# paritybit-ai/XFL

Measured on AMD Instinct MI355X. Metric: 2048-bit Paillier encrypts/s (device-resident), higher is better.
Workload: dtype u32; 1 GPU; DJN private-key (CRT) encrypt, obfuscated, precision 7, 1000000 float64 plaintexts/GPU resident in HBM; key_bits=2048, elements_per_gpu=1000000, fixed_base_window_bits=23, fixed_base_window_split=False, parallelism=shard1, table_bytes=193273528320

## Files before the change

__graft_entry__.py:

```python
import os
import sys

ROOT = os.path.dirname(os.path.abspath(__file__))
if ROOT not in sys.path:
    sys.path.insert(0, ROOT)


def build() -> None:
    from xfl_amd import build as b
    b.build()
    from oracle import build as ob
    ob.build()
    import runpy
    for script in ("build.py", "build_redc_block.py"):
        try:
            runpy.run_path(os.path.join(ROOT, "tests", "native", script), run_name="tests_native_build")["build"]()
        except Exception as exc:
            print(f"warning: device self-test harnesses not built ({script}): {exc}", file=sys.stderr)
    import xfl_amd
    from xfl_amd import _native
    _native.lib()


def smoke() -> None:
    import numpy as np

    from oracle import paillier_oracle as O
    from xfl_amd import _native as nat
    from xfl_amd.paillier.utils import getprimeover
    import random
    import math

    rng = random.Random(7)
    while True:
        p, q = getprimeover(1024, rng=rng), getprimeover(1024, rng=rng)
        if p != q and math.gcd(p - 1, q - 1) == 2:
            break
    n = p * q
    x = rng.getrandbits(n.bit_length()) | (1 << (n.bit_length() - 1))
    h = pow(-(x * x), n, n * n)
    dk = nat.DeviceKey(2048, n, p, q, h, device=0)
    ok = O.derive_private(p, q, h)
    vals = np.random.default_rng(0).standard_normal(64) * 10
    ms = [O.encode_element(ok, float(v), 7)[0] for v in vals]
    rs = [rng.randrange(1, ok["djn_exp_bound"]) for _ in vals]
    ct = nat.words_to_ints(dk.encrypt_words(nat.ints_to_words(ms, dk.nw), nat.ints_to_words(rs, dk.rand_words)))
    want = [O.encrypt_m(ok, m, r) for m, r in zip(ms, rs)]
# ... 11 lines not shown
```

xfl_amd/csrc/keyconst.hpp:

```cpp
#pragma once
#include <algorithm>
#include <cstdint>
#include <stdexcept>
#include <utility>
#include <vector>

#include "hostbn.hpp"
#include "keydev.hpp"
#include "rns_layout.hpp"

namespace xhe {

struct ModSpec {
  int S, W;
  int S4() const { return (S + 3) & ~3; }
  BigU R() const { return pow2((size_t)W * S); }
};

struct KeySpec {
  int K;
  bool priv, djn;
  ModSpec mp2, mp2L, mp2X;
  ModSpec mp;
  ModSpec mn2, mn2X;
// ... 194 lines not shown
  }
  if (sq) {
    if (ns >= P_SCHED_MAX) throw std::runtime_error("rns schedule overflow");
    v[P_SCHED + ns++] = sq << 8;
  }
  v[P_NS] = (uint32_t)ns;
  return v;
}
}

using RowF = const uint32_t* KeyDev::*;
using PairF = const uint2* KeyDev::*;
using ModF = ModDev KeyDev::*;
using IntF = int KeyDev::*;

struct Dst {
  RowF w = nullptr;
  PairF d = nullptr;
  ModF m = nullptr;
  const uint32_t* ModDev::*mw = nullptr;
  size_t* off = nullptr;
  Dst(RowF f) : w(f) {}
  Dst(PairF f) : d(f) {}
  Dst(ModF mod, const uint32_t* ModDev::*f) : m(mod), mw(f) {}
  Dst(size_t* o) : off(o) {}
};

struct KeyImage {
  std::vector<uint32_t> words;
  KeyDev kd{};
  int rand_bits = 0, rand_words = 0;
  size_t hM_n2 = 0, hM_p2[2] = {0, 0};
  std::vector<uint32_t> hinvM_p[2];

  void put(const std::vector<uint32_t>& v, Dst dst, size_t min_words = 0) {
    const size_t off = words.size();
    const size_t len = (std::max(v.size(), min_words) + 3) & ~(size_t)3;
    words.resize(off + len, 0u);
    std::copy(v.begin(), v.end(), words.begin() + off);
    if (dst.off) *dst.off = off;
    else binds.push_back({dst, off});
  }
  void put_limbs(const BigU& x, const ModSpec& s, Dst dst) { put(x.to_limbs(s.W, s.S), dst, s.S4()); }
  void put_words(const BigU& x, int nw, Dst dst) {
    std::vector<uint32_t> v(nw);
    x.to_words(v.data(), nw);
    put(v, dst);
  }
  void put_mod(const BigU& M, const ModSpec& s, ModF m, int npow = 0) {
    const BigU R1 = mod(s.R(), M), R2 = mulmod(R1, R1, M), R3 = mulmod(R2, R1, M);
    put_limbs(M, s, {m, &ModDev::N});
    put_limbs(R1, s, {m, &ModDev::R1});
    put_limbs(R2, s, {m, &ModDev::R2});
    put_limbs(R3, s, {m, &ModDev::R3});
    (kd.*m).n0inv = mont_ninv(M.word(0), s.W);
    if (npow <= 0) return;
    std::vector<uint32_t> rows((size_t)npow * s.S4(), 0u);
    BigU x = mod(BigU(1), M);
    for (int j = 0; j < npow; ++j) {
      const std::vector<uint32_t> l = x.to_limbs(s.W, s.S);
      std::copy(l.begin(), l.end(), rows.begin() + (size_t)j * s.S4());
      x = mulmod(x, R1, M);
    }
    put(rows, {m, &ModDev::Rpow});
  }

// ... 180 lines not shown
      const BigU &X = pr[i].X, RX = mod(s.pmd.R(), X), R2 = mulmod(RX, RX, X);
      im.put_limbs(mulmod(mod(pr[i].Y, X), mulmod(R2, R2, X), X), s.pmd, pq::mu[i]);
    }
}

inline void pdigit_constants(KeyImage& im, const KeySpec& s, const Prime& pr, int i) {
  const BigU &X = pr.X, &X2 = pr.X2;
  const DigitMod d(X, s.pd);
  digit_modulus(im, d, X2, pq::dm[i], pq::x_kn2[i], pq::x_rmn[i]);
  im.put(mask_plus_e(X, d.RM, d.s), pq::x_topc[i]);
  im.put_limbs(mulmod(mod(pr.Y, X), mulmod(mulmod(d.RM, d.RM, X), d.RM, X), X), d.s, pq::x_fold[i]);
  const BigU Rx2 = mod(d.R, X2), R2 = mulmod(Rx2, Rx2, X2), R4 = mulmod(R2, R2, X2);
  im.put(digit_pairs(d, mulmod(R4, modinv(mod(s.mp2.R(), X2), X2), X2)), pq::x_dwt[i]);
  im.put(digit_pairs(d, R4), pq::x_dw[i]);
  im.put_limbs(mulmod(pr.h, d.RM, X), d.s, pq::x_hpR[i]);
}

inline void exponent_constants(KeyImage& im, const KeySpec& s, const BigU& n, const Prime (&pr)[2]) {
  im.put_limbs(shl(pr[0].X, 1), s.mp, &KeyDev::p2x_lim);
  im.put_limbs(pr[0].X, s.mp, &KeyDev::p_lim);
  for (int i = 0; i < 2; ++i) {
    const BigU e = mod(n, mul(pr[i].X, sub(pr[i].X, BigU(1))));
    im.kd.*pq::e_bits[i] = (int)e.bits();
    im.put_words(e, s.nw(), pq::e_words[i]);
  }
}

inline std::vector<uint32_t> inverse_base_limbs(const ModSpec& s, const BigU& h, const BigU& P) {
  std::vector<uint32_t> v = mulmod(modinv(mod(h, P), P), mod(s.R(), P), P).to_limbs(s.W, s.S);
  v.resize((size_t)s.S4(), 0u);
  return v;
}

inline KeyImage derive_key_constants(const KeySpec& s, const BigU& n, const BigU* p, const BigU* q, const BigU* h) {
  KeyImage im;
  KeyDev& kd = im.kd;
  kd.K = s.K;
  kd.nw = s.nw();
  kd.n2w = s.n2w();
  kd.priv = s.priv;
  kd.djn = s.djn;
  kd.n_bits = (int)n.bits();
  im.rand_bits = s.djn ? (int)(n.bits() / 2) : (int)n.bits();
  im.rand_words = (im.rand_bits + 31) / 32;
  if (s.djn) {
    kd.win = s.win;
    win_layout(im.rand_bits, s.win, s.priv && s.split, &kd.nwin, &kd.nhi);
  }
  const BigU n2 = mul(n, n);
  n2_constants(im, s, n, n2, s.djn && !s.priv ? h : nullptr);
  if (s.K == 2048) {
    kd.ndig = 1;
    ndigit_constants(im, s, n, n2);
  }
  if (!s.priv) return im;
  Prime pr[2] = {{*p, *q, mul(*p, *p), {}, {}}, {*q, *p, mul(*q, *q), {}, {}}};
  for (Prime& x : pr) x.n = mod(n, x.X2);
  prime2_constants(im, s, pr, h, kd.nwin);
  decrypt_constants(im, s, n, pr);
  if (s.K != 2048) {
    kd.pmdx_dec = 1;
    for (int i = 0; i < 2; ++i) pdigit_constants(im, s, pr[i], i);
  }
  exponent_constants(im, s, n, pr);
  if (s.K == 2048 && s.djn)
    for (int i = 0; i < 2; ++i) im.hinvM_p[i] = inverse_base_limbs(s.pmd, *h, pr[i].X);
  return im;
}

}
```

xfl_amd/csrc/pdigit_dev.hpp:

```cpp
#pragma once
#include "bn_dev.hpp"

namespace xhe {

struct PmdLdsQ {
  const uint32_t* q;
  XHE_DEV uint4 load4(int i) const { return *reinterpret_cast<const uint4*>(q + (i >> 2) * 256); }
};

template <int K_>
struct PMD {
  static constexpr int K = K_, W = 28, BL = 6;
  static constexpr int NQ = (2 * K + 3) / 4;
  static constexpr uint32_t MASK = (1u << W) - 1u;
  static_assert((K - 1) % BL == 0, "positions 1..K-1 in blocks of 6");
  static_assert((double)(3 * K + 2) * (double)(1ull << 57) < 18446744073709551616.0, "accumulator bound");

  uint32_t p[K];
  uint32_t n0inv;

  XHE_DEV void init(const uint32_t* __restrict__ P, uint32_t ninv) {
#pragma unroll
    for (int j = 0; j < K; ++j) p[j] = __builtin_amdgcn_readfirstlane(P[j]);
    n0inv = ninv;
// ... 532 lines not shown
  for (int j = 0; j < K; ++j) br = ((int64_t)r[j] - (int64_t)M.p[j] + br) >> 28;
  const bool ge = br == 0;
  br = 0;
#pragma unroll
  for (int j = 0; j < K; ++j) {
    const int64_t v = (int64_t)r[j] - (int64_t)(ge ? M.p[j] : 0u) + br;
    r[j] = (uint32_t)v & ((1u << 28) - 1u);
    br = v >> 28;
  }
  return ge;
}

template <int K>
XHE_DEV void pmd_mod_small(const PMD<K>& M, uint32_t (&m)[K]) {
  constexpr uint32_t MASK = PMD<K>::MASK;
  const uint32_t mt = (m[K - 1] << 4) | (m[K - 2] >> 24);
  const uint32_t pt = (M.p[K - 1] << 4) | (M.p[K - 2] >> 24);
  const uint32_t q = mt / (pt + 1u);
  uint64_t cy = 0;
  int64_t br = 0;
#pragma unroll
  for (int j = 0; j < K; ++j) {
    const uint64_t qp = (uint64_t)q * M.p[j] + cy;
    cy = qp >> 28;
    const int64_t v = (int64_t)m[j] - (int64_t)(qp & MASK) + br;
    m[j] = (uint32_t)v & MASK;
    br = v >> 28;
  }
#pragma unroll
  for (int t = 0; t < 3; ++t) pmd_csub<K>(M, m);
}

template <int K>
XHE_DEV void pmd_from_mont2(const PMD<K>& M, const uint32_t (&X)[2 * K], const uint32_t* RmodP, uint32_t (&e)[K],
                            uint32_t (&f)[K]) {
  uint32_t m[K];
  {
    uint64_t T[2 * K];
#pragma unroll
    for (int j = 0; j < 2 * K; ++j) T[j] = X[j];
    pmd_redc_wide<K>(M, T, e, m);
  }
  __builtin_amdgcn_sched_barrier(0);
  const bool ge = pmd_csub<K>(M, e);
  __builtin_amdgcn_sched_barrier(0);
  pmd_mod_small<K>(M, m);
  __builtin_amdgcn_sched_barrier(0);
  int64_t br = 0;
#pragma unroll
  for (int j = 0; j < K; ++j) {
    const int64_t v = (int64_t)(ge ? RmodP[j] : 0u) - (int64_t)m[j] + br;
    f[j] = (uint32_t)v & ((1u << 28) - 1u);
    br = v >> 28;
  }
  if (br) {
    int64_t cy = 0;
#pragma unroll
    for (int j = 0; j < K; ++j) {
      const int64_t v = (int64_t)f[j] + (int64_t)M.p[j] + cy;
      f[j] = (uint32_t)v & ((1u << 28) - 1u);
      cy = v >> 28;
    }
  }
}

template <int K, int RW>
// ... 647 lines not shown
```

xfl_amd/csrc/xhe.hip:

```cpp
#include <hip/hip_runtime.h>
#include <stdint.h>
#include <stdlib.h>
#include <string.h>

#include <chrono>
#include <cmath>
#include <cstdio>
#include <memory>
#include <mutex>
#include <atomic>
#include <stdexcept>
#include <unordered_map>
#include <utility>
#include <string>
#include <type_traits>
#include <vector>

#include "../../include/xhe.h"
#include "abi_common.hpp"
#include "hostbn.hpp"
#include "keyconst.hpp"
#include "paths.hpp"
#include "xhe_kernels.hpp"
#include "fermat_dev.hpp"
// ... 132 lines not shown
}

}

struct xhe_key {
  int device = 0;
  int K = 0, nw = 0, n2w = 0;
  bool priv = false, djn = false;
  int rand_bits = 0, rand_words = 0;
  uint32_t* d_blob = nullptr;
  uint32_t* d_tab = nullptr;
  KeyDev kd{};
  std::vector<uint32_t> n_host;
  std::vector<uint32_t> n2_host;
  int n_bits = 0;
  int dneg = 0;
};

namespace {

struct DevGuard {
  int prev = -1;
  explicit DevGuard(int dev) {
    HIPCHK(hipGetDevice(&prev));
    if (prev != dev) HIPCHK(hipSetDevice(dev));
  }
  ~DevGuard() {
    if (prev >= 0) (void)hipSetDevice(prev);
  }
};

template <class MP2, int RW>
void build_tables_m(xhe_key* k, const ModDev& md, const uint32_t* d_hM, uint32_t* d_tab, uint32_t* d_chain,
                    uint32_t* d_ws, hipStream_t s);

int64_t chain_rows_h(int win) { return ((int64_t)1 << (win / 2)) + ((int64_t)1 << (win - win / 2)); }

template <class MP2, int RW>
void build_tables_sync(xhe_key* k, const ModDev* md, const uint32_t* const* d_hM, uint32_t* const* d_tab, int count) {
  hipStream_t st[2] = {nullptr, nullptr};
  uint32_t* ws[2] = {nullptr, nullptr};
  uint32_t* chain[2] = {nullptr, nullptr};
  const int win = k->kd.win, nwin = k->kd.nwin, nhi = k->kd.nhi;
  const size_t chain_words =
      (size_t)std::max<int64_t>(nhi ? (nhi + 1) * chain_rows_h(win + 1) : 0, (nwin - nhi) * chain_rows_h(win)) *
      MP2::S4;
  for (int i = 0; i < count; ++i) {
    HIPCHK(hipStreamCreateWithFlags(&st[i], hipStreamNonBlocking));
    HIPCHK(hipMalloc(&ws[i], MP2::S4 * sizeof(uint32_t) * 4));
    HIPCHK(hipMalloc(&chain[i], chain_words * sizeof(uint32_t)));
    build_tables_m<MP2, RW>(k, md[i], d_hM[i], d_tab[i], chain[i], ws[i], st[i]);
  }
  for (int i = 0; i < count; ++i) {
    HIPCHK(hipStreamSynchronize(st[i]));
    HIPCHK(hipFree(ws[i]));
    HIPCHK(hipFree(chain[i]));
    HIPCHK(hipStreamDestroy(st[i]));
  }
}

template <class MP2>
void build_chains_seg(const ModDev& md, const uint32_t* d_base, int win, int nwin, int nbases, uint32_t* d_chain,
                      uint32_t* d_ws, hipStream_t s) {
  const int half = win / 2;
  launch(k_tab_bases<MP2>, dim3(1), dim3(64), s, md, d_base, win, nbases, d_chain, d_ws);
  auto blocks = [&](int64_t groups) { return dim3((unsigned)std::max<int64_t>(1, (groups * MP2::TPI + 255) / 256)); };
  launch(k_tab_one<MP2>, blocks(nwin), dim3(256), s, md, win, nwin, d_chain);
  const int lim_lo = (1 << half) + 1, lim_hi = 1 << (win - half);
  for (int t = 0; (1 << t) < lim_lo - 1; ++t) {
    launch(k_tab_level<MP2>, blocks((int64_t)nwin << t), dim3(256), s, md, md.N, win, nwin, t, 0, lim_lo, d_chain);
  }
  for (int t = 0; (1 << t) < lim_hi - 1; ++t) {
    launch(k_tab_level<MP2>, blocks((int64_t)nwin << t), dim3(256), s, md, md.N, win, nwin, t, half, lim_hi, d_chain);
  }
}

template <class MP2, int RW>
void build_tables_seg(const ModDev& md, const uint32_t* d_base, int win, int nwin, int nbases, uint32_t* d_tab,
                      int64_t rs, uint32_t* d_chain, uint32_t* d_ws, hipStream_t s) {
  build_chains_seg<MP2>(md, d_base, win, nwin, nbases, d_chain, d_ws, s);
  auto blocks = [&](int64_t groups) { return dim3((unsigned)std::max<int64_t>(1, (groups * MP2::TPI + 255) / 256)); };
  int64_t rows = (int64_t)nwin << win;
  launch((k_tab_combine<MP2, RW>), blocks(rows), dim3(256), s, md, md.N, win, nwin, d_chain, d_tab, rs);
}

template <class MP2, int RW>
void build_tables_m(xhe_key* k, const ModDev& md, const uint32_t* d_hM, uint32_t* d_tab, uint32_t* d_chain,
                    uint32_t* d_ws, hipStream_t s) {
  const int win = k->kd.win, nwin = k->kd.nwin, nhi = k->kd.nhi;
  const int64_t rs = RW == k->K / 32 ? k->kd.tab_rs : RW;
  if (nhi == 0) {
    build_tables_seg<MP2, RW>(md, d_hM, win, nwin, nwin, d_tab, rs, d_chain, d_ws, s);
    return;
  }
  uint32_t* base2 = d_ws + 2 * MP2::S4;
  build_tables_seg<MP2, RW>(md, d_hM, win + 1, nhi, nhi + 1, d_tab, rs, d_chain, d_ws, s);
  HIPCHK(hipMemcpyAsync(base2, d_chain + ((size_t)nhi * chain_rows_h(win + 1) + 1) * MP2::S4,
                        MP2::S4 * sizeof(uint32_t), hipMemcpyDeviceToDevice, s));
  build_tables_seg<MP2, RW>(md, base2, win, nwin - nhi, nwin - nhi, d_tab + ((size_t)nhi << (win + 1)) * rs, rs,
                            d_chain, d_ws, s);
}

template <class M>
size_t inv_chain_words(const KeyDev& kd) {
  return (size_t)(kd.nhi * chain_rows_h(kd.win + 1) + (kd.nwin - kd.nhi) * chain_rows_h(kd.win)) * M::S4;
}
template <class M>
void build_chains_m(const KeyDev& kd, const ModDev& md, const uint32_t* d_hM, uint32_t* d_chain, uint32_t* d_ws,
                    hipStream_t s) {
  const int win = kd.win, nwin = kd.nwin, nhi = kd.nhi;
  if (nhi == 0) {
    build_chains_seg<M>(md, d_hM, win, nwin, nwin, d_chain, d_ws, s);
    return;
  }
  uint32_t* base2 = d_ws + 2 * M::S4;
  uint32_t* narrow = d_chain + (size_t)nhi * chain_rows_h(win + 1) * M::S4;
  build_chains_seg<M>(md, d_hM, win + 1, nhi, nhi + 1, d_chain, d_ws, s);
  HIPCHK(hipMemcpyAsync(base2, narrow + M::S4, M::S4 * sizeof(uint32_t), hipMemcpyDeviceToDevice, s));
  build_chains_seg<M>(md, base2, win, nwin - nhi, nwin - nhi, narrow, d_ws, s);
}

template <class Sh>
KeySpec key_spec(const xhe_key* k, int win) {
  KeySpec s{};
  s.K = Sh::K;
  s.priv = k->priv;
  s.djn = k->djn;
  s.win = win & 0xff;
  s.split = (win & XHE_WIN_SPLIT) != 0;
  s.mp2 = {Sh::MP2::S, Sh::MP2::W};
  s.mp2L = {Sh::MP2L::S, Sh::MP2L::W};
  s.mp2X = {Sh::MP2X::S, Sh::MP2X::W};
  s.mp = {Sh::MP::S, Sh::MP::W};
// ... 14 lines not shown
  return s;
}

int64_t table_rows(const KeyDev& kd) { return (int64_t)(kd.nwin + kd.nhi) << kd.win; }

template <class F>
void rows_to_digits(int64_t rows, int tpr, unsigned block, int ntab, F&& launch_one) {
  const dim3 grid((unsigned)((rows * tpr + block - 1) / block));
  for (int i = 0; i < ntab; ++i) launch_one(i, grid, dim3(block));
  HIPCHK(hipDeviceSynchronize());
}

void build_private_tables(xhe_key* k, const KeyImage& im) {
  KeyDev& kd = k->kd;
  const int64_t rows = table_rows(kd);
  const size_t tab_words = (size_t)rows * (size_t)(k->K / 32);
  HIPCHK(hipMalloc(&k->d_tab, 2 * tab_words * sizeof(uint32_t)));
  kd.tab_rs = k->K / 32;
  kd.tab_p2 = k->d_tab;
  kd.tab_q2 = k->d_tab + tab_words;
  const ModDev mds[2] = {kd.p2, kd.q2};
  const uint32_t* hms[2] = {k->d_blob + im.hM_p2[0], k->d_blob + im.hM_p2[1]};
  uint32_t* tabs[2] = {k->d_tab, k->d_tab + tab_words};
  with_shape(k->K, [&](auto sh) {
    using Sh = decltype(sh);
    if constexpr (Sh::K == 2048) {
      using MP = typename Sh::MP;
      const ModDev mp[2] = {kd.p, kd.q};
      hipStream_t st[2];
      uint32_t *inv[2], *ws[2];
      for (int i = 0; i < 2; ++i) {
        HIPCHK(hipStreamCreateWithFlags(&st[i], hipStreamNonBlocking));
        HIPCHK(hipMalloc(&inv[i], inv_chain_words<MP>(kd) * sizeof(uint32_t)));
        HIPCHK(hipMalloc(&ws[i], MP::S4 * sizeof(uint32_t) * 4));
        uint32_t* base = ws[i] + 3 * MP::S4;
        HIPCHK(hipMemcpy(base, im.hinvM_p[i].data(), MP::S4 * sizeof(uint32_t), hipMemcpyHostToDevice));
        build_chains_m<MP>(kd, mp[i], base, inv[i], ws[i], st[i]);
      }
      build_tables_sync<typename Sh::MP2, Sh::RW>(k, mds, hms, tabs, 2);
      for (int i = 0; i < 2; ++i) HIPCHK(hipStreamSynchronize(st[i]));
      kd.pmd = 1;
      rows_to_digits(rows, 1, 256, 2, [&](int i, dim3 grid, dim3 block) {
        launch((k_tab_to_pmd<MP, Sh::RW>), grid, block, nullptr, mp[i], mp[i].N, inv[i], kd.win, kd.nhi, tabs[i], rows,
               (int64_t)kd.tab_rs);
      });
      for (int i = 0; i < 2; ++i) {
        HIPCHK(hipFree(inv[i]));
        HIPCHK(hipFree(ws[i]));
        HIPCHK(hipStreamDestroy(st[i]));
      }
    } else {
      build_tables_sync<typename Sh::MP2, Sh::RW>(k, mds, hms, tabs, 2);
      kd.pmdx = 1;
      using D = typename Sh::PDXO;
      rows_to_digits(rows, D::TPI, 128, 2, [&](int i, dim3 grid, dim3 block) {
        launch((k_tab_to_pmdx<D, Sh::RW>), grid, block, nullptr, kd, i, tabs[i], rows, (int64_t)kd.tab_rs);
      });
    }
  });
}

void build_public_tables(xhe_key* k, const KeyImage& im) {
  KeyDev& kd = k->kd;
  const int64_t rows = table_rows(kd);
  HIPCHK(hipMalloc(&k->d_tab, (size_t)rows * (size_t)(k->K / 16) * sizeof(uint32_t)));
  kd.tab_n2 = k->d_tab;
  const uint32_t* hm = k->d_blob + im.hM_n2;
  uint32_t* tab = k->d_tab;
  with_shape(k->K, [&](auto sh) {
    using Sh = decltype(sh);
    build_tables_sync<typename Sh::MN2, Sh::RW2>(k, &kd.n2, &hm, &tab, 1);
    if constexpr (Sh::K == 2048) {
      if (!pins().ndig_pub) return;
      kd.pub_nd = 1;
      rows_to_digits(rows, ND2048::TPI, 128, 1, [&](int, dim3 grid, dim3 block) {
        launch((k_tab_to_pmdx<ND2048, Sh::RW2>), grid, block, nullptr, kd, 2, tab, rows, (int64_t)Sh::RW2);
// ... 195 lines not shown

template <class Sh, class MP2 = typename Sh::MP2>
void crt_enc_launch(const xhe_key* k, int64_t n, uint32_t* ws, uint32_t* ct, hipStream_t s) {
  const int blocks = (int)((n * MP2::TPI + 255) / 256);
  if constexpr (MP2::TPI == 1)
    launch((k_crt_enc_w<MP2, 2 * Sh::K / 32>), dim3(blocks), dim3(256), s, k->kd, k->kd.p2.N, n, ws, ct);
  else
    launch(k_crt_enc<MP2>, dim3(blocks), dim3(256), s, k->kd, k->kd.p2.N, n, ws, ct);
}

template <class Sh>
void encrypt_impl(const xhe_key* k, const uint32_t* m, const uint32_t* r, int64_t count, uint32_t* ct, hipStream_t s) {
  using MP2 = typename Sh::MP2;
  int64_t chunk = std::min<int64_t>(count, kChunk);
  WsScope wsc(s);
  uint32_t* ws = wsc.get<uint32_t>((size_t)2 * 2 * MP2::S4 * chunk * sizeof(uint32_t));
  uint2* xst = nullptr;
  uint32_t *xrows = nullptr, *xwords = nullptr;
  for (int64_t off = 0; off < count; off += chunk) {
    int64_t n = std::min(chunk, count - off);
    switch (paths::enc_djn(Sh::K, MP2::TPI, k->kd.pmd, k->kd.pmdx, n, pins())) {
      case paths::EncDjn::PMD:
        if constexpr (Sh::K == 2048) {
          ProfScope ps("k_djn_pmd", s);
          const int G = paths::pmd_split(n, pins());
          const dim3 grid((unsigned)((n * G + 127) / 128), 2);
          auto run = [&](auto kern) {
            launch(kern, grid, dim3(128), s, k->kd, k->kd.p.N, k->kd.q.N, k->kd.p2.N, k->kd.q2.N,
                   m + (size_t)off * k->nw, r + (size_t)off * k->rand_words, k->rand_words, n, ws);
          };
          if (G == 16) run(k_djn_pmd<MP2, 37, Sh::RW, 16>);
          else if (G == 4) run(k_djn_pmd<MP2, 37, Sh::RW, 4>);
          else run(k_djn_pmd<MP2, 37, Sh::RW, 1>);
          crt_enc_launch<Sh>(k, n, ws, ct + (size_t)off * k->n2w, s);
          continue;
        } else no_path("encrypt (k_djn_pmd)");
      case paths::EncDjn::PMDX:
        if constexpr (Sh::K != 2048) {
          using D = typename Sh::PDX;
          if (!xst) {
            xst = wsc.get<uint2>((size_t)2 * D::K * chunk * sizeof(uint2));
            xrows = wsc.get<uint32_t>((size_t)2 * 2 * Sh::PDXO::MN::S4 * chunk * sizeof(uint32_t));
            xwords = wsc.get<uint32_t>((size_t)2 * chunk * Sh::RW * sizeof(uint32_t));
          }
          const dim3 g4((unsigned)((n * D::TPI + 127) / 128), 2);
          {
            ProfScope ps("k_djn_pmdx", s);
            launch((k_djn_pmdx<D, Sh::RW>), g4, dim3(128), s, k->kd, r + (size_t)off * k->rand_words, k->rand_words, n,
                   xst);
          }
          using DO = typename Sh::PDXO;
          launch((k_pmdx_enc_out<DO, Sh::RW>), dim3((unsigned)((n * DO::TPI + 127) / 128), 2), dim3(128), s, k->kd,
                 m + (size_t)off * k->nw, n, xst, xrows, xwords);
          launch(k_words_to_rows<MP2>, dim3((unsigned)((n * MP2::TPI + 255) / 256), 2), dim3(256), s, xwords, Sh::RW,
                 n, ws);
          crt_enc_launch<Sh>(k, n, ws, ct + (size_t)off * k->n2w, s);
          continue;
        } else no_path("encrypt (k_djn_pmdx)");
      case paths::EncDjn::POW_X: {
        using MX = typename Sh::MP2X;
        launch((k_djn_pow_x<MX, MP2::S4, Sh::RW>), dim3((unsigned)((n * MX::TPI + 255) / 256), 2), dim3(256), s, k->kd,
               m + (size_t)off * k->nw, r + (size_t)off * k->rand_words, k->rand_words, n, ws);
        break;
      }
      case paths::EncDjn::POW_LDS:
        if constexpr (MP2::TPI == 1) {
          ProfScope ps("k_djn_pow_lds", s);
// ... 1702 lines not shown
```

xfl_amd/csrc/xhe_kernels.hpp:

```cpp
#pragma once
#include "bn_dev.hpp"
#include "keydev.hpp"
#include "pdigit_dev.hpp"

#include <type_traits>

namespace xhe {

enum : int32_t { ST_OK = 0, ST_OVERFLOW = 1, ST_VALUE = 2 };

struct EncVal {
  int32_t st, e;
  int neg, w;
  uint32_t v0, v1, v2;
};

XHE_DEV EncVal encode_value(double v, int mode, int e0, int has_max, int max_exp) {
  EncVal r{ST_OK, 0, 0, 0, 0u, 0u, 0u};
  uint64_t bits = __double_as_longlong(v);
  r.neg = (int)(bits >> 63);
  int bexp = (int)((bits >> 52) & 0x7FF);
  uint64_t frac = bits & ((1ull << 52) - 1);
  int e;
  if (mode == 0) {
// ... 530 lines not shown
    }
#pragma unroll
    for (int j = 0; j < KP; ++j) c[j] = 0u;
  }
  for (int w = g + G; w < key.nwin; w += G) {
    stage(w);
    M.mul_row(a, c, slot, topc);
  }
  if constexpr (G > 1) {
#pragma unroll
    for (int s = 1; s < G; s <<= 1) {
      const bool writer = (g & (2 * s - 1)) == s && g < key.nwin;
      const bool reader = (g & (2 * s - 1)) == 0 && g + s < key.nwin;
      if (reader) D::lam_add_slot(slot, slot + 4 * s);
      wave_sync_mem_();
      if (writer) {
#pragma unroll
        for (int q = 0; q < D::NQ; ++q)
          *reinterpret_cast<uint4*>(slot + q * 256) =
              make_uint4(2 * q < KP ? a[2 * q] : 0u, 2 * q < KP ? c[2 * q] : 0u, 2 * q + 1 < KP ? a[2 * q + 1] : 0u,
                         2 * q + 1 < KP ? c[2 * q + 1] : 0u);
      }
      wave_sync_mem_();
      if (reader) M.mul(a, c, slot + 4 * s, topc);
      wave_sync_mem_();
    }
    if (g != 0) return;
  }
  M.finish(a, c, slot, prime ? Pq : Pp);
  __builtin_amdgcn_sched_barrier(0);
  uint32_t b[MP2::L];
  M.to_mont2(a, c, b);
  __builtin_amdgcn_sched_barrier(0);
  MP2 N;
  N.init(prime ? Nq2 : Np2, prime ? key.q2.n0inv : key.p2.n0inv);
  N.redc_wide(b, AZero{});
  N.reduce_once(b);
  const int64_t eo = ((int64_t)blockIdx.x * blockDim.x + (uint32_t)opaque_i((int)threadIdx.x)) / G;
  N.store_strided(b, ws + (size_t)prime * 2 * MP2::S4 * count + eo, (int)count);
}

template <int KP>
XHE_DEV void pmd_pow_uniform(const PMD<KP>& M, uint32_t (&a)[KP], uint32_t (&c)[KP], const uint32_t* ex, int ebits,
                             uint4* __restrict__ tab_base, int lane, int G, uint32_t* slot, const uint32_t* topc) {
  constexpr int NQ = PMD<KP>::NQ;
#define tab (tab_base + opaque_i(lane))
  auto quad = [&](int q) -> uint4 {
    return make_uint4(2 * q < KP ? a[2 * q] : 0u, 2 * q < KP ? c[2 * q] : 0u, 2 * q + 1 < KP ? a[2 * q + 1] : 0u,
                      2 * q + 1 < KP ? c[2 * q + 1] : 0u);
  };
  auto put_slot = [&]() XHE_INL {
#pragma unroll
    for (int q = 0; q < NQ; ++q) *reinterpret_cast<uint4*>(slot + q * 256) = quad(q);
  };
  auto put_tab = [&](int t) XHE_INL {
#pragma unroll
    for (int q = 0; q < NQ; ++q) tab[((size_t)t * NQ + q) * G] = quad(q);
  };
  auto tab_to_slot = [&](int t) XHE_INL {
    uint4 v[NQ];
#pragma unroll
    for (int q = 0; q < NQ; ++q) v[q] = tab[((size_t)t * NQ + q) * G];
#pragma unroll
    for (int q = 0; q < NQ; ++q) *reinterpret_cast<uint4*>(slot + q * 256) = v[q];
  };
  auto tab_to_regs = [&](int t) XHE_INL {
#pragma unroll
    for (int q = 0; q < NQ; ++q) {
      const uint4 v = tab[((size_t)t * NQ + q) * G];
// ... 578 lines not shown
    wave_sync_mem_();
  };
  auto emit = [&](uint32_t limb) XHE_INL {
    acc |= (uint64_t)limb << nb;
    nb += W;
    if (nb >= 32 && w < NW2) {
      ring[lane * RS + (w & 63)] = (uint32_t)acc;
      acc >>= 32;
      nb -= 32;
      ++w;
      if ((w & 31) == 0) flush((w - 32) & 63);
    }
  };
  for (int i0 = 0; i0 < MP2::S4; i0 += 4) {
    const uint4 a4 = ARow{key.q2_lim}.load4(i0);
#pragma unroll
    for (int r = 0; r < 4; ++r) {
      if (i0 + r < S) {
        const uint32_t ai = comp4(a4, r);
        const uint64_t x0 = mad64(ai, b[0], T[0]);
        mad_shift(T, b, ai);
        T[S - 1] = 0;
        T[0] += x0 >> W;
        emit((uint32_t)x0 & MP2::MASK);
      }
    }
  }
  uint32_t hi[S];
  M.normalize(T, hi);
#pragma unroll
  for (int j = 0; j < S; ++j) emit(hi[j]);
}

template <class MP2>
__global__ void __launch_bounds__(256, 2) k_raw_enc(KeyDev key, const uint32_t* __restrict__ m_words, int64_t count,
                                                    uint32_t* __restrict__ ws, uint32_t* __restrict__ out) {
  const int64_t e = ((int64_t)blockIdx.x * blockDim.x + threadIdx.x) / MP2::TPI;
  if (e >= count) return;
  const int st = (int)count;
  uint32_t* row = ws + e;
  MP2 M;
  M.init(key.p2.N, 0);
  uint32_t b[MP2::L];
  M.load_words(b, m_words + (size_t)e * key.nw, key.nw);
  {
    const int g = MP2::G::g();
#pragma unroll
    for (int j = 0; j < MP2::L; ++j) row[(size_t)(g * MP2::L + j) * st] = (g == 0 && j == 0) ? 1u : 0u;
  }
  wave_sync_mem_();
  M.wide_mul_add_store(b, ARow{key.n_lim}, row, st, out + (size_t)e * key.n2w, key.n2w);
}

template <class MP2>
XHE_DEV void pow_uniform_exp(const MP2& M, uint32_t (&b)[MP2::L], const uint32_t* ex, int ebits,
                             uint32_t* tab, uint32_t* sq, int st, uint32_t* sq_lds = nullptr) {
  const size_t rs = (size_t)MP2::S4 * st;
  auto square = [&]() XHE_INL {
    if constexpr (MP2::kSqr) {
      if (sq_lds) {
        M.sqr(b, SqLds<MP2>(sq_lds));
        return;
      }
    }
    if (sq_lds) {
      const SqLds<MP2> L(sq_lds);
// ... 868 lines not shown
  const int w = (int)(((int64_t)blockIdx.x * blockDim.x + threadIdx.x) / MP2::TPI);
  if (w >= nwin) return;
  MP2 M;
  M.init(md.N, md.n0inv);
  uint32_t b[MP2::L];
  M.load_row(b, md.R1);
  M.reduce_once(b);
  M.store_row(b, chain + (size_t)w * chain_rows(win) * MP2::S4);
}

template <class MP2>
__global__ void __launch_bounds__(256, 2) k_tab_level(ModDev md, const uint32_t* __restrict__ Nm, int win, int nwin,
                                                       int t, int sh, int lim, uint32_t* __restrict__ chain) {
  const int64_t idx = ((int64_t)blockIdx.x * blockDim.x + threadIdx.x) / MP2::TPI;
  const int64_t per = (int64_t)1 << t;
  if (idx >= (int64_t)nwin * per) return;
  const int w = (int)(idx >> t);
  const int64_t d = per + 1 + (idx & (per - 1));
  if (d >= lim) return;
  const int half = win / 2;
  uint32_t* cw = chain + (size_t)w * chain_rows(win) * MP2::S4;
  MP2 M;
  M.init(Nm, md.n0inv);
  uint32_t b[MP2::L];
  M.load_row(b, cw + (size_t)chain_index(d - per, sh, half) * MP2::S4);
  M.mul(b, ARow{cw + (size_t)chain_index(per, sh, half) * MP2::S4});
  M.reduce_once(b);
  M.store_row(b, cw + (size_t)chain_index(d, sh, half) * MP2::S4);
}

template <class MP2, int RW>
__global__ void __launch_bounds__(256, 2) k_tab_combine(ModDev md, const uint32_t* __restrict__ Nm, int win,
                                                         int nwin, const uint32_t* __restrict__ chain,
                                                         uint32_t* __restrict__ tab, int64_t rs) {
  __shared__ __attribute__((aligned(16))) uint32_t sc_all[(256 / MP2::TPI) * MP2::S4];
  const int64_t idx = ((int64_t)blockIdx.x * blockDim.x + threadIdx.x) / MP2::TPI;
  const int64_t rows = (int64_t)nwin << win;
  if (idx >= rows) return;
  const int half = win / 2;
  const int w = (int)(idx >> win);
  const int d = (int)(idx & ((1 << win) - 1));
  const int lo = d & ((1 << half) - 1), hi = d >> half;
  const uint32_t* cw = chain + (size_t)w * chain_rows(win) * MP2::S4;
  MP2 M;
  M.init(Nm, md.n0inv);
  uint32_t b[MP2::L];
  if (hi == 0) {
    M.load_row(b, cw + (size_t)chain_index(lo, 0, half) * MP2::S4);
  } else if (lo == 0) {
    M.load_row(b, cw + (size_t)chain_index(hi, half, half) * MP2::S4);
  } else {
    M.load_row(b, cw + (size_t)chain_index(hi, half, half) * MP2::S4);
    M.mul(b, ARow{cw + (size_t)chain_index(lo, 0, half) * MP2::S4});
    M.reduce_once(b);
  }
  uint32_t* sc = sc_all + (size_t)((threadIdx.x % 256) / MP2::TPI) * MP2::S4;
  M.store_row(b, sc);
  wave_sync_mem_();
  pack_words_<MP2::W, MP2::TPI>(sc, 1, MP2::S, tab + (size_t)idx * rs, RW);
}

template <class MP, int RW>
__global__ void __launch_bounds__(256, 2) k_tab_to_pmd(ModDev mp, const uint32_t* __restrict__ P,
                                                       const uint32_t* __restrict__ inv, int win, int nhi,
                                                       uint32_t* __restrict__ tab, int64_t rows, int64_t rs) {
  static_assert(MP::TPI == 1 && MP::W == 28, "one lane per row on the digit limbs");
  constexpr int KP = MP::S;
  const int64_t r = (int64_t)blockIdx.x * blockDim.x + threadIdx.x;
  if (r >= rows) return;
  uint32_t* row = tab + (size_t)r * rs;
  uint32_t w[RW];
#pragma unroll
  for (int q = 0; q < RW / 4; ++q) {
    const uint4 v = reinterpret_cast<const uint4*>(row)[q];
    w[4 * q] = v.x, w[4 * q + 1] = v.y, w[4 * q + 2] = v.z, w[4 * q + 3] = v.w;
  }
  uint32_t X[2 * KP];
#pragma unroll
  for (int l = 0; l < 2 * KP; ++l) {
    const int bit = 28 * l, k = bit >> 5, sh = bit & 31;
    const uint32_t lo = word_or0(w, k, RW), hi = word_or0(w, k + 1, RW);
    X[l] = __builtin_amdgcn_alignbit(hi, lo, sh) & ((1u << 28) - 1u);
  }
  PMD<KP> M;
  M.init(P, mp.n0inv);
  uint32_t e[KP], f[KP];
  pmd_from_mont2<KP>(M, X, mp.R1, e, f);
  __builtin_amdgcn_sched_barrier(0);
  {
    const int64_t wide = (int64_t)nhi << (win + 1);
    const bool hiw = r < wide;
    const int wb = win + (hiw ? 1 : 0), half = wb / 2;
    const int64_t rr = hiw ? r : r - wide;
    const int64_t d = rr & (((int64_t)1 << wb) - 1);
    const uint32_t* cw = inv + ((size_t)(rr >> wb) * chain_rows(wb) + (hiw ? 0 : (size_t)nhi * chain_rows(win + 1))) * MP::S4;
    const int64_t lo = d & (((int64_t)1 << half) - 1), hi = d >> half;
    MP N;
    N.init(P, mp.n0inv);
    N.mul(f, ARow{cw + (size_t)(hi ? chain_index(hi, half, half) : 0) * MP::S4});
    N.reduce_once(f);
    N.mul(f, ARow{cw + (size_t)chain_index(lo, 0, half) * MP::S4});
    N.reduce_once(f);
  }
  auto word = [&](const uint32_t (&l)[KP], int k) -> uint32_t {
    const int bit = 32 * k, j = bit / 28, sh = bit - 28 * j;
    uint64_t v = (uint64_t)l[j] >> sh;
    if (j + 1 < KP) v |= (uint64_t)l[j + 1] << (28 - sh);
    if (j + 2 < KP) v |= (uint64_t)l[j + 2] << (56 - sh);
    return (uint32_t)v;
  };
#pragma unroll
  for (int q = 0; q < RW / 8; ++q) {
    reinterpret_cast<uint4*>(row)[q] = make_uint4(word(e, 4 * q), word(e, 4 * q + 1), word(e, 4 * q + 2), word(e, 4 * q + 3));
    reinterpret_cast<uint4*>(row)[RW / 8 + q] =
        make_uint4(word(f, 4 * q), word(f, 4 * q + 1), word(f, 4 * q + 2), word(f, 4 * q + 3));
  }
}

XHE_DEV void magwin_push(uint32_t w4[4], uint32_t& low_or, int& hk, uint32_t w, int k) {
  if (!w) return;
  const int g = k - hk;
#pragma unroll
  for (int t = 0; t < 4; ++t)
    if (t < g) low_or |= w4[t];
  uint32_t nw4[4];
#pragma unroll
  for (int t = 0; t < 4; ++t) nw4[t] = t == 3 ? w : (t + g <= 3 ? w4[t + g] : 0u);
#pragma unroll
  for (int t = 0; t < 4; ++t) w4[t] = nw4[t];
  hk = k;
}

XHE_DEV void magwin_round53(const uint32_t w4[4], uint32_t low_or, int hk, int bl, bool rne, uint64_t& mant,
                            int& shift) {
  auto magw = [&](int k) -> uint32_t {
// ... 174 lines not shown
```

Before: 51.08 million encrypts/s.

## Fold CRT recombination constants into tables and use symmetric CRT combine kernel

Precomputes CRT coefficients (inverse of the other prime squared) and folds them into the first window row of the fixed-base tables and their inverse digit tables, so the per-residue results already carry the CRT scaling. The per-element Montgomery exit reduction is replaced by a cheap quotient-estimate reduction, and the final CRT recombination becomes a new kernel computing u*q^2 + v*p^2 with a single conditional subtraction of n^2, using LDS staging for coalesced output. The aim is to remove the multiplications and reductions of the old CRT combine. It adds table-build complexity and relies on carefully argued bounds for the partial reductions.

```diff
diff --git a/__graft_entry__.py b/__graft_entry__.py
--- a/__graft_entry__.py
+++ b/__graft_entry__.py
@@ -12,7 +12,7 @@
     from oracle import build as ob
     ob.build()
     import runpy
-    for script in ("build.py", "build_redc_block.py"):
+    for script in ("build.py", "build_redc_block.py", "build_exit_reduce.py"):
         try:
             runpy.run_path(os.path.join(ROOT, "tests", "native", script), run_name="tests_native_build")["build"]()
         except Exception as exc:
diff --git a/xfl_amd/csrc/keyconst.hpp b/xfl_amd/csrc/keyconst.hpp
--- a/xfl_amd/csrc/keyconst.hpp
+++ b/xfl_amd/csrc/keyconst.hpp
@@ -250,6 +250,7 @@
   int rand_bits = 0, rand_words = 0;
   size_t hM_n2 = 0, hM_p2[2] = {0, 0};
   std::vector<uint32_t> hinvM_p[2];
+  std::vector<uint32_t> crtC_p2[2], crtCinv_p[2];
 
   void put(const std::vector<uint32_t>& v, Dst dst, size_t min_words = 0) {
     const size_t off = words.size();
@@ -496,6 +497,15 @@
   return v;
 }
 
+inline void crt_fold_limbs(const KeySpec& s, const Prime& pr, std::vector<uint32_t>& cM, std::vector<uint32_t>& cinvM) {
+  const BigU Y2 = mod(mul(pr.Y, pr.Y), pr.X2);
+  cM = modinv(Y2, pr.X2).to_limbs(s.mp2.W, s.mp2.S);
+  cM.resize((size_t)s.mp2.S4(), 0u);
+  const BigU &X = pr.X, R2 = mod(s.mp2.R(), X), R = mod(s.pmd.R(), X);
+  cinvM = mulmod(mod(Y2, X), mulmod(R2, R, X), X).to_limbs(s.pmd.W, s.pmd.S);
+  cinvM.resize((size_t)s.pmd.S4(), 0u);
+}
+
 inline KeyImage derive_key_constants(const KeySpec& s, const BigU& n, const BigU* p, const BigU* q, const BigU* h) {
   KeyImage im;
   KeyDev& kd = im.kd;
@@ -528,7 +538,10 @@
   }
   exponent_constants(im, s, n, pr);
   if (s.K == 2048 && s.djn)
-    for (int i = 0; i < 2; ++i) im.hinvM_p[i] = inverse_base_limbs(s.pmd, *h, pr[i].X);
+    for (int i = 0; i < 2; ++i) {
+      im.hinvM_p[i] = inverse_base_limbs(s.pmd, *h, pr[i].X);
+      crt_fold_limbs(s, pr[i], im.crtC_p2[i], im.crtCinv_p[i]);
+    }
   return im;
 }
 
diff --git a/xfl_amd/csrc/pdigit_dev.hpp b/xfl_amd/csrc/pdigit_dev.hpp
--- a/xfl_amd/csrc/pdigit_dev.hpp
+++ b/xfl_amd/csrc/pdigit_dev.hpp
@@ -588,6 +588,26 @@
 }
 
 template <int K>
+XHE_DEV void pmd_exit_reduce(uint32_t (&V)[2 * K], const uint32_t* __restrict__ N2) {
+  static_assert(K == 37, "the tops are taken at bit 2016 = 28 * 72 of a 2048-bit P^2");
+  constexpr int S = 2 * K;
+  constexpr uint32_t MASK = PMD<K>::MASK;
+  const uint64_t vt = ((uint64_t)V[S - 1] << 28) | V[S - 2];
+  const uint32_t pt = (N2[S - 1] << 28) | N2[S - 2];
+  const uint32_t qh = (uint32_t)((double)vt / ((double)pt + 1.0));
+  uint64_t cy = 0;
+  int64_t br = 0;
+#pragma unroll
+  for (int j = 0; j < S; ++j) {
+    const uint64_t qp = mad64s(qh, N2[j], cy);
+    cy = qp >> 28;
+    const int64_t v = (int64_t)V[j] - (int64_t)(qp & MASK) + br;
+    V[j] = j + 1 < S ? ((uint32_t)v & MASK) : (uint32_t)v;
+    br = v >> 28;
+  }
+}
+
+template <int K>
 XHE_DEV void pmd_from_mont2(const PMD<K>& M, const uint32_t (&X)[2 * K], const uint32_t* RmodP, uint32_t (&e)[K],
                             uint32_t (&f)[K]) {
   uint32_t m[K];
diff --git a/xfl_amd/csrc/xhe.hip b/xfl_amd/csrc/xhe.hip
--- a/xfl_amd/csrc/xhe.hip
+++ b/xfl_amd/csrc/xhe.hip
@@ -188,12 +188,13 @@
 
 template <class MP2, int RW>
 void build_tables_m(xhe_key* k, const ModDev& md, const uint32_t* d_hM, uint32_t* d_tab, uint32_t* d_chain,
-                    uint32_t* d_ws, hipStream_t s);
+                    uint32_t* d_ws, hipStream_t s, const uint32_t* d_c0);
 
 int64_t chain_rows_h(int win) { return ((int64_t)1 << (win / 2)) + ((int64_t)1 << (win - win / 2)); }
 
 template <class MP2, int RW>
-void build_tables_sync(xhe_key* k, const ModDev* md, const uint32_t* const* d_hM, uint32_t* const* d_tab, int count) {
+void build_tables_sync(xhe_key* k, const ModDev* md, const uint32_t* const* d_hM, uint32_t* const* d_tab, int count,
+                       const uint32_t* const* d_c0 = nullptr) {
   hipStream_t st[2] = {nullptr, nullptr};
   uint32_t* ws[2] = {nullptr, nullptr};
   uint32_t* chain[2] = {nullptr, nullptr};
@@ -205,7 +206,7 @@
     HIPCHK(hipStreamCreateWithFlags(&st[i], hipStreamNonBlocking));
     HIPCHK(hipMalloc(&ws[i], MP2::S4 * sizeof(uint32_t) * 4));
     HIPCHK(hipMalloc(&chain[i], chain_words * sizeof(uint32_t)));
-    build_tables_m<MP2, RW>(k, md[i], d_hM[i], d_tab[i], chain[i], ws[i], st[i]);
+    build_tables_m<MP2, RW>(k, md[i], d_hM[i], d_tab[i], chain[i], ws[i], st[i], d_c0 ? d_c0[i] : nullptr);
   }
   for (int i = 0; i < count; ++i) {
     HIPCHK(hipStreamSynchronize(st[i]));
@@ -233,28 +234,28 @@
 
 template <class MP2, int RW>
 void build_tables_seg(const ModDev& md, const uint32_t* d_base, int win, int nwin, int nbases, uint32_t* d_tab,
-                      int64_t rs, uint32_t* d_chain, uint32_t* d_ws, hipStream_t s) {
+                      int64_t rs, uint32_t* d_chain, uint32_t* d_ws, hipStream_t s, const uint32_t* d_c0) {
   build_chains_seg<MP2>(md, d_base, win, nwin, nbases, d_chain, d_ws, s);
   auto blocks = [&](int64_t groups) { return dim3((unsigned)std::max<int64_t>(1, (groups * MP2::TPI + 255) / 256)); };
   int64_t rows = (int64_t)nwin << win;
-  launch((k_tab_combine<MP2, RW>), blocks(rows), dim3(256), s, md, md.N, win, nwin, d_chain, d_tab, rs);
+  launch((k_tab_combine<MP2, RW>), blocks(rows), dim3(256), s, md, md.N, win, nwin, d_chain, d_tab, rs, d_c0);
 }
 
 template <class MP2, int RW>
 void build_tables_m(xhe_key* k, const ModDev& md, const uint32_t* d_hM, uint32_t* d_tab, uint32_t* d_chain,
-                    uint32_t* d_ws, hipStream_t s) {
+                    uint32_t* d_ws, hipStream_t s, const uint32_t* d_c0) {
   const int win = k->kd.win, nwin = k->kd.nwin, nhi = k->kd.nhi;
   const int64_t rs = RW == k->K / 32 ? k->kd.tab_rs : RW;
   if (nhi == 0) {
-    build_tables_seg<MP2, RW>(md, d_hM, win, nwin, nwin, d_tab, rs, d_chain, d_ws, s);
+    build_tables_seg<MP2, RW>(md, d_hM, win, nwin, nwin, d_tab, rs, d_chain, d_ws, s, d_c0);
     return;
   }
   uint32_t* base2 = d_ws + 2 * MP2::S4;
-  build_tables_seg<MP2, RW>(md, d_hM, win + 1, nhi, nhi + 1, d_tab, rs, d_chain, d_ws, s);
+  build_tables_seg<MP2, RW>(md, d_hM, win + 1, nhi, nhi + 1, d_tab, rs, d_chain, d_ws, s, d_c0);
   HIPCHK(hipMemcpyAsync(base2, d_chain + ((size_t)nhi * chain_rows_h(win + 1) + 1) * MP2::S4,
                         MP2::S4 * sizeof(uint32_t), hipMemcpyDeviceToDevice, s));
   build_tables_seg<MP2, RW>(md, base2, win, nwin - nhi, nwin - nhi, d_tab + ((size_t)nhi << (win + 1)) * rs, rs,
-                            d_chain, d_ws, s);
+                            d_chain, d_ws, s, nullptr);
 }
 
 template <class M>
@@ -335,16 +336,20 @@
       for (int i = 0; i < 2; ++i) {
         HIPCHK(hipStreamCreateWithFlags(&st[i], hipStreamNonBlocking));
         HIPCHK(hipMalloc(&inv[i], inv_chain_words<MP>(kd) * sizeof(uint32_t)));
-        HIPCHK(hipMalloc(&ws[i], MP::S4 * sizeof(uint32_t) * 4));
+        HIPCHK(hipMalloc(&ws[i], (MP::S4 * 5 + Sh::MP2::S4) * sizeof(uint32_t)));
         uint32_t* base = ws[i] + 3 * MP::S4;
         HIPCHK(hipMemcpy(base, im.hinvM_p[i].data(), MP::S4 * sizeof(uint32_t), hipMemcpyHostToDevice));
+        HIPCHK(hipMemcpy(ws[i] + 4 * MP::S4, im.crtCinv_p[i].data(), MP::S4 * sizeof(uint32_t), hipMemcpyHostToDevice));
+        HIPCHK(hipMemcpy(ws[i] + 5 * MP::S4, im.crtC_p2[i].data(), Sh::MP2::S4 * sizeof(uint32_t), hipMemcpyHostToDevice));
         build_chains_m<MP>(kd, mp[i], base, inv[i], ws[i], st[i]);
       }
-      build_tables_sync<typename Sh::MP2, Sh::RW>(k, mds, hms, tabs, 2);
+      const uint32_t* c0[2] = {ws[0] + 5 * MP::S4, ws[1] + 5 * MP::S4};
+      build_tables_sync<typename Sh::MP2, Sh::RW>(k, mds, hms, tabs, 2, c0);
       for (int i = 0; i < 2; ++i) HIPCHK(hipStreamSynchronize(st[i]));
       kd.pmd = 1;
       rows_to_digits(rows, 1, 256, 2, [&](int i, dim3 grid, dim3 block) {
-        launch((k_tab_to_pmd<MP, Sh::RW>), grid, block, nullptr, mp[i], mp[i].N, inv[i], kd.win, kd.nhi, tabs[i], rows,
+        launch((k_tab_to_pmd<MP, Sh::RW>), grid, block, nullptr, mp[i], mp[i].N, inv[i], ws[i] + 4 * MP::S4, kd.win,
+               kd.nhi, tabs[i], rows,
                (int64_t)kd.tab_rs);
       });
       for (int i = 0; i < 2; ++i) {
@@ -606,7 +611,8 @@
           if (G == 16) run(k_djn_pmd<MP2, 37, Sh::RW, 16>);
           else if (G == 4) run(k_djn_pmd<MP2, 37, Sh::RW, 4>);
           else run(k_djn_pmd<MP2, 37, Sh::RW, 1>);
-          crt_enc_launch<Sh>(k, n, ws, ct + (size_t)off * k->n2w, s);
+          launch((k_crt_sym_w<MP2, 2 * Sh::K / 32>), dim3((unsigned)((n + 255) / 256)), dim3(256), s, k->kd,
+                 k->kd.p2.N, k->kd.q2.N, n, ws, ct + (size_t)off * k->n2w);
           continue;
         } else no_path("encrypt (k_djn_pmd)");
       case paths::EncDjn::PMDX:
diff --git a/xfl_amd/csrc/xhe_kernels.hpp b/xfl_amd/csrc/xhe_kernels.hpp
--- a/xfl_amd/csrc/xhe_kernels.hpp
+++ b/xfl_amd/csrc/xhe_kernels.hpp
@@ -586,9 +586,9 @@
   uint32_t b[MP2::L];
   M.to_mont2(a, c, b);
   __builtin_amdgcn_sched_barrier(0);
+  pmd_exit_reduce<KP>(b, prime ? Nq2 : Np2);
   MP2 N;
   N.init(prime ? Nq2 : Np2, prime ? key.q2.n0inv : key.p2.n0inv);
-  N.redc_wide(b, AZero{});
   N.reduce_once(b);
   const int64_t eo = ((int64_t)blockIdx.x * blockDim.x + (uint32_t)opaque_i((int)threadIdx.x)) / G;
   N.store_strided(b, ws + (size_t)prime * 2 * MP2::S4 * count + eo, (int)count);
@@ -1233,6 +1233,115 @@
   for (int j = 0; j < S; ++j) emit(hi[j]);
 }
 
+template <int N>
+XHE_DEV void mad2s_shift6(uint64_t (&T)[N], uint32_t u, uint32_t v, const uint32_t* __restrict__ A,
+                          const uint32_t* __restrict__ B, int j) {
+  asm("v_mad_u64_u32 %0, vcc, %7, %9, %1\n\t"
+      "v_mad_u64_u32 %1, vcc, %7, %10, %2\n\t"
+      "v_mad_u64_u32 %2, vcc, %7, %11, %3\n\t"
+      "v_mad_u64_u32 %3, vcc, %7, %12, %4\n\t"
+      "v_mad_u64_u32 %4, vcc, %7, %13, %5\n\t"
+      "v_mad_u64_u32 %5, vcc, %7, %14, %6\n\t"
+      "v_mad_u64_u32 %0, vcc, %8, %15, %0\n\t"
+      "v_mad_u64_u32 %1, vcc, %8, %16, %1\n\t"
+      "v_mad_u64_u32 %2, vcc, %8, %17, %2\n\t"
+      "v_mad_u64_u32 %3, vcc, %8, %18, %3\n\t"
+      "v_mad_u64_u32 %4, vcc, %8, %19, %4\n\t"
+      "v_mad_u64_u32 %5, vcc, %8, %20, %5"
+      : "+v"(T[j - 1]), "+v"(T[j]), "+v"(T[j + 1]), "+v"(T[j + 2]), "+v"(T[j + 3]), "+v"(T[j + 4])
+      : "v"(T[j + 5]), "v"(u), "v"(v), "s"(A[j]), "s"(A[j + 1]), "s"(A[j + 2]), "s"(A[j + 3]), "s"(A[j + 4]),
+        "s"(A[j + 5]), "s"(B[j]), "s"(B[j + 1]), "s"(B[j + 2]), "s"(B[j + 3]), "s"(B[j + 4]), "s"(B[j + 5])
+      : "vcc");
+}
+
+template <class MP2, int NW2>
+__global__ void __launch_bounds__(256, 2) k_crt_sym_w(KeyDev key, const uint32_t* __restrict__ Np2,
+                                                      const uint32_t* __restrict__ Nq2, int64_t count,
+                                                      const uint32_t* __restrict__ ws, uint32_t* __restrict__ out) {
+  static_assert(MP2::TPI == 1, "one lane per residue");
+  constexpr int S = MP2::S, W = MP2::W, RS = S + 1;
+  static_assert(NW2 % 32 == 0 && 2 * S * W >= 32 * NW2 + 1, "ciphertext words and the bit above them");
+  static_assert(S >= 64 && (RS & 1) == 1, "the ring (64 words) inside a lane's row; odd stride: no bank conflicts");
+  static_assert((S - 2) % 6 == 0, "positions 1..S-2 in blocks of 6, position S-1 alone");
+  static_assert((double)(2 * S) * (double)((1ull << W) - 1) * (double)((1ull << W) - 1) + (double)(1ull << (64 - W)) <
+                    18446744073709551616.0,
+                "column bound: 2 S products and a carry");
+  __shared__ uint32_t img_all[4][64 * RS];
+  const int64_t e = (int64_t)blockIdx.x * blockDim.x + threadIdx.x;
+  const int lane = (int)(threadIdx.x & 63);
+  uint32_t* ring = img_all[(threadIdx.x >> 6) & 3];
+  uint32_t* mine = ring + lane * RS;
+  const int64_t e0 = e - lane;
+  if (e0 >= count) return;
+  const int64_t ec = e < count ? e : count - 1;
+  const size_t st = (size_t)count;
+  const uint32_t* up = ws + ec;
+  const uint32_t* uq = ws + (size_t)2 * MP2::S4 * count + ec;
+  uint64_t T[S];
+#pragma unroll
+  for (int j = 0; j < S; ++j) T[j] = 0;
+  uint32_t u1 = up[0], v1 = uq[0], u2 = up[st], v2 = uq[st];
+#pragma unroll 1
+  for (int i = 0; i < S; ++i) {
+    const uint32_t u = u1, v = v1;
+    u1 = u2, v1 = v2;
+    const size_t in = (size_t)(i + 2 < S ? i + 2 : S - 1) * st;
+    u2 = up[in], v2 = uq[in];
+    const uint64_t x0 = mad64s(v, Np2[0], mad64s(u, Nq2[0], T[0]));
+#pragma unroll
+    for (int j = 1; j + 6 <= S - 1; j += 6) mad2s_shift6(T, u, v, Nq2, Np2, j);
+    T[S - 2] = mad64s(v, Np2[S - 1], mad64s(u, Nq2[S - 1], 0ull));
+    T[0] += x0 >> W;
+    mine[i] = (uint32_t)x0 & MP2::MASK;
+  }
+  uint32_t hi[S];
+  MP2 M;
+  M.init(Np2, key.p2.n0inv);
+  M.normalize(T, hi);
+  auto walk = [&](auto&& fn) XHE_INL -> uint32_t {
+    uint64_t acc = 0;
+    int nb = 0, w = 0;
+    auto limb = [&](uint32_t l) XHE_INL {
+      acc |= (uint64_t)l << nb;
+      nb += W;
+      if (nb >= 32) {
+        fn(w, (uint32_t)acc);
+        acc >>= 32;
+        nb -= 32;
+        ++w;
+      }
+    };
+#pragma unroll 1
+    for (int j = 0; j < S; ++j) limb(mine[j]);
+#pragma unroll
+    for (int j = 0; j < S; ++j) limb(hi[j]);
+    return (uint32_t)acc;
+  };
+  uint32_t br = 0, top = 0;
+  const uint32_t rest = walk([&](int w, uint32_t x) XHE_INL {
+    if (w < NW2) br = (uint32_t)(((uint64_t)x - key.n2_words[w] - br) >> 63);
+    else top |= x;
+  });
+  const bool ge = (top | rest) != 0u || br == 0u;
+  br = 0;
+  walk([&](int w, uint32_t x) XHE_INL {
+    if (w >= NW2) return;
+    const uint64_t d = (uint64_t)x - (ge ? key.n2_words[w] : 0u) - br;
+    br = (uint32_t)(d >> 63);
+    mine[w & 63] = (uint32_t)d;
+    if (((w + 1) & 31) == 0) {
+      const int base = (w + 1 - 32) & 63;
+      wave_sync_mem_();
+#pragma unroll 4
+      for (int r = 0; r < 32; ++r) {
+        const int el = 2 * r + (lane >> 5), wd = lane & 31;
+        if (e0 + el < count) out[(size_t)(e0 + el) * NW2 + (w + 1 - 32) + wd] = ring[el * RS + base + wd];
+      }
+      wave_sync_mem_();
+    }
+  });
+}
+
 template <class MP2>
 __global__ void __launch_bounds__(256, 2) k_raw_enc(KeyDev key, const uint32_t* __restrict__ m_words, int64_t count,
                                                     uint32_t* __restrict__ ws, uint32_t* __restrict__ out) {
@@ -2167,7 +2276,8 @@
 template <class MP2, int RW>
 __global__ void __launch_bounds__(256, 2) k_tab_combine(ModDev md, const uint32_t* __restrict__ Nm, int win,
                                                          int nwin, const uint32_t* __restrict__ chain,
-                                                         uint32_t* __restrict__ tab, int64_t rs) {
+                                                         uint32_t* __restrict__ tab, int64_t rs,
+                                                         const uint32_t* __restrict__ c0) {
   __shared__ __attribute__((aligned(16))) uint32_t sc_all[(256 / MP2::TPI) * MP2::S4];
   const int64_t idx = ((int64_t)blockIdx.x * blockDim.x + threadIdx.x) / MP2::TPI;
   const int64_t rows = (int64_t)nwin << win;
@@ -2189,6 +2299,10 @@
     M.mul(b, ARow{cw + (size_t)chain_index(lo, 0, half) * MP2::S4});
     M.reduce_once(b);
   }
+  if (c0 && w == 0) {
+    M.mul(b, ARow{c0});
+    M.reduce_once(b);
+  }
   uint32_t* sc = sc_all + (size_t)((threadIdx.x % 256) / MP2::TPI) * MP2::S4;
   M.store_row(b, sc);
   wave_sync_mem_();
@@ -2197,7 +2311,8 @@
 
 template <class MP, int RW>
 __global__ void __launch_bounds__(256, 2) k_tab_to_pmd(ModDev mp, const uint32_t* __restrict__ P,
-                                                       const uint32_t* __restrict__ inv, int win, int nhi,
+                                                       const uint32_t* __restrict__ inv,
+                                                       const uint32_t* __restrict__ cinv, int win, int nhi,
                                                        uint32_t* __restrict__ tab, int64_t rows, int64_t rs) {
   static_assert(MP::TPI == 1 && MP::W == 28, "one lane per row on the digit limbs");
   constexpr int KP = MP::S;
@@ -2236,6 +2351,10 @@
     N.reduce_once(f);
     N.mul(f, ARow{cw + (size_t)chain_index(lo, 0, half) * MP::S4});
     N.reduce_once(f);
+    if (r < ((int64_t)1 << (win + (nhi ? 1 : 0)))) {
+      N.mul(f, ARow{cinv});
+      N.reduce_once(f);
+    }
   }
   auto word = [&](const uint32_t (&l)[KP], int k) -> uint32_t {
     const int bit = 32 * k, j = bit / 28, sh = bit - 28 * j;
```

New measurement: 50.64 million encrypts/s. Within noise of the previous version (-0.9%).
